# liannuaa/GenPC

Measured on AMD Instinct MI355X. Metric: chamfer_nn_pair_dist_throughput, higher is better.
Workload: dtype f32; 1 GPU; chamfer_3DDist.forward B=1 N=M=16384 (both directions), one pair per rank; points=16384, batch=1, arith=fma

## Files before the change

genpc_amd/csrc/nn.h:

```cpp
#pragma once
#include "common.h"
#include "grid.h"
#include "nn_plan.h"
#include "nn_decode.h"
#include "nn_ragged_dense_plan.h"

namespace genpc {

constexpr int kWavesPerBlock = kBlock / kWave;

struct NNDir {
    const unsigned *dupmask;
    float *tmaxp;
    unsigned long long *part;
    const float *q;
    const float *t;
    float *out_d;
    int *out_i;
    const uint4 *arec;
    int block_begin;
    int dup_shared;
    NNDiv by_qblocks;
    int qblocks;
    int nq, nt;
    int slices;
    int fin_begin;
    NNDiv by_fblocks;
    int ntmax;
    int unit_begin;
    int ntp;
};

struct NNArgs {
    NNDir dir[2];
    int slice_len;
    NNDiv by_b;
    int ndir;
    int b;
    int debug;
    int hint_stride;
    NNDiv by_hint;
    int fma;
    unsigned long long *stats;
    unsigned *hint;
    int *arrive;
    float radius2;
};

#define NN_GLOBAL(T) __attribute__((address_space(1))) T *
#define NN_CONST(p) ((const __attribute__((address_space(4))) float *)(p))
#define NN_ARG(T, name, field) T name##_0 = a.dir[0].field, name##_1 = a.dir[1].field
#define NN_ARG_PTR(T, name, field) NN_GLOBAL(T) name##_0 = (NN_GLOBAL(T))a.dir[0].field; NN_GLOBAL(T) name##_1 = (NN_GLOBAL(T))a.dir[1].field
#define NN_HELD(name) "+s"(name##_0), "+s"(name##_1)
#define NN_OF_DIR(name) (d ? name##_1 : name##_0)

typedef float f32x16 __attribute__((ext_vector_type(16)));

struct Top3 {
    float a1, a2, a3;
    int c1, c2;
};

__device__ __forceinline__ void top3_init(Top3 &s)
{
    s.a1 = s.a2 = s.a3 = __builtin_inff();
    s.c1 = s.c2 = -1;
}

__device__ __forceinline__ void top3_insert(Top3 &s, float m, int id)
{
    asm("v_cmp_lt_f32 vcc, %[m], %[a2]\n\t"
        "v_cndmask_b32 %[c2], %[c2], %[id], vcc\n\t"
        "v_cmp_lt_f32 vcc, %[m], %[a1]\n\t"
        "v_cndmask_b32 %[c2], %[c2], %[c1], vcc\n\t"
        "v_cndmask_b32 %[c1], %[c1], %[id], vcc\n\t"
        "v_med3_f32 %[a3], %[a2], %[a3], %[m]\n\t"
        "v_med3_f32 %[a2], %[a1], %[a2], %[m]\n\t"
        "v_min_f32 %[a1], %[a1], %[m]"
        : [a1] "+v"(s.a1), [a2] "+v"(s.a2), [a3] "+v"(s.a3), [c1] "+v"(s.c1), [c2] "+v"(s.c2)
        : [m] "v"(m), [id] "v"(id)
        : "vcc");
}

__device__ __forceinline__ unsigned list_enc(float base, float v)
{
    if (!(v < __builtin_inff())) return v != v ? 0xffffu : 0xff00u;
    const float s = fmaxf(fabsf(base), fabsf(v)) * 4.76837158203125e-07f;
    const float d = (v - base) - s;
    if (!(d > 0.0f)) return 0u;
    return (__float_as_uint(d) >> 15) & 0xffffu;
}
__device__ __forceinline__ float list_dec(float base, unsigned code) { return base + __uint_as_float(code << 15); }

typedef unsigned long long ListRec __attribute__((ext_vector_type(2)));
template <typename P>
__device__ __forceinline__ auto list_rec(P *part, int list, size_t bnq, int batch, int nq, int j)
{
    typedef typename std::conditional<std::is_const<P>::value, const ListRec, ListRec>::type R;
    return (R *)part + ((size_t)list * bnq + (size_t)batch * nq + j);
}

template <int FMA, int LEN>
__device__ __forceinline__ void rescan_chunk(const float *__restrict__ T, int nt, int base, float qx, float qy,
                                             float qz, float &bd, int &bi)
{
    typedef float f4u __attribute__((ext_vector_type(4), aligned(4)));
    bd = __builtin_inff();
    bi = base;
    if (base + LEN <= nt) {
        const f4u *tp = (const f4u *)(T + (size_t)base * 3);
#pragma unroll
        for (int c8 = LEN - 8; c8 >= 0; c8 -= 8) {
            f4u v[6];
#pragma unroll
            for (int i = 0; i < 6; i++) v[i] = tp[(c8 >> 2) * 3 + i];
            const float f[24] = {v[0].x, v[0].y, v[0].z, v[0].w, v[1].x, v[1].y, v[1].z, v[1].w,
                                 v[2].x, v[2].y, v[2].z, v[2].w, v[3].x, v[3].y, v[3].z, v[3].w,
                                 v[4].x, v[4].y, v[4].z, v[4].w, v[5].x, v[5].y, v[5].z, v[5].w};
#pragma unroll
            for (int c = 7; c >= 0; c--) {
                const float dd = sqdist<FMA>(f[c * 3 + 0] - qx, f[c * 3 + 1] - qy, f[c * 3 + 2] - qz);
                const bool le = dd <= bd;
                bd = le ? dd : bd;
                bi = le ? base + c8 + c : bi;
            }
        }
    } else {
        for (int c = LEN - 1; c >= 0; c--) {
            int kk = base + c;
            kk = kk < nt ? kk : nt - 1;
            const float *tp = T + (size_t)kk * 3;
            const float dd = sqdist<FMA>(tp[0] - qx, tp[1] - qy, tp[2] - qz);
            const bool le = dd <= bd;
            bd = le ? dd : bd;
            bi = le ? kk : bi;
        }
    }
}

__device__ __forceinline__ int tile_row(int w) { return 8 * ((w >> 2) & 3) + 4 * (w >> 4) + (w & 3); }

constexpr int kRefTile = 512;

__device__ __forceinline__ int block_or(int v, int *s)
{
    static_assert(kWavesPerBlock * kWave == kBlock, "block_or folds one word per wave of a kBlock-thread block");
    const int any = __ballot(v != 0) != 0ull;
    __syncthreads();
    if ((threadIdx.x & (kWave - 1)) == 0) s[threadIdx.x >> 6] = any;
    __syncthreads();
    int r = 0;
#pragma unroll
    for (int w = 0; w < kWavesPerBlock; w++) r |= s[w];
    return r;
}
template <int FMA>
__device__ __forceinline__ void nn_exhaustive(const float *__restrict__ Qp, const float *__restrict__ T, int nt, int j,
                                              float *__restrict__ od, int *__restrict__ oi, float *s_red, int *s_fi)
{
    const int lane = threadIdx.x & (kWave - 1), wave = threadIdx.x >> 6;
    const float x = Qp[(size_t)j * 3 + 0], y = Qp[(size_t)j * 3 + 1], z = Qp[(size_t)j * 3 + 2];
    int dead = 0;
    for (int k = threadIdx.x * kRefTile; k < nt; k += kBlock * kRefTile) {
        const float *tp = T + (size_t)k * 3;
        const float hd = sqdist<FMA>(tp[0] - x, tp[1] - y, tp[2] - z);
        dead |= hd != hd;
    }
    dead = block_or(dead, s_fi);
    float bd = __builtin_inff();
    int bi = 0x7fffffff;
    if (!dead) {
        for (int k = threadIdx.x; k < nt; k += kBlock) {
            const float *tp = T + (size_t)k * 3;
            const float dd = sqdist<FMA>(tp[0] - x, tp[1] - y, tp[2] - z);
            const bool lt = dd < bd;
            bd = lt ? dd : bd;
            bi = lt ? k : bi;
        }
    } else {
        for (int k = threadIdx.x; k < nt; k += kBlock) {
            const float *hp = T + (size_t)(k & ~(kRefTile - 1)) * 3;
            const float hd = sqdist<FMA>(hp[0] - x, hp[1] - y, hp[2] - z);
            const float *tp = T + (size_t)k * 3;
            const float dd = sqdist<FMA>(tp[0] - x, tp[1] - y, tp[2] - z);
            const bool lt = dd < bd && hd == hd;
            bd = lt ? dd : bd;
            bi = lt ? k : bi;
        }
    }
#pragma unroll
    for (int o = 32; o >= 1; o >>= 1) {
        const float obd = __shfl_xor(bd, o);
        const int obi = __shfl_xor(bi, o);
        const bool other = obd < bd || (obd == bd && obi < bi);
        bd = other ? obd : bd;
        bi = other ? obi : bi;
    }
    __syncthreads();
    if (lane == 0) { s_red[wave] = bd; s_fi[wave] = bi; }
    __syncthreads();
    if (threadIdx.x == 0) {
        for (int w = 1; w < kWavesPerBlock; w++) {
            const bool other = s_red[w] < bd || (s_red[w] == bd && s_fi[w] < bi);
            bd = other ? s_red[w] : bd;
            bi = other ? s_fi[w] : bi;
        }
        const float d0 = sqdist<FMA>(T[0] - x, T[1] - y, T[2] - z);
        if (d0 != d0 || bi == 0x7fffffff) {
            bd = d0;
            bi = 0;
        }
        od[j] = bd;
        oi[j] = bi;
    }
}

__device__ __forceinline__ float nn_tau(float a_best, float qq, float tmax2, double kQT, double kTT)
{
    const double u = 1.01 * 5.9604644775390625e-8;
    const double T = sqrt((double)tmax2), qn = sqrt((double)qq);
    const double kSub = 64.0 * 1.401298464324817e-45;
    const double E1 = u * (kQT * qn * T + kTT * T * T + 3.0 * (double)qq) + kSub;
    const double eta = u * (qn + T);
    double up = (double)a_best + (double)qq + E1;
    up = sqrt(up > 0.0 ? up : 0.0) + eta;
    up = up * up * (1.0 + 6.0 * u) + kSub;
    double r = sqrt(up / (1.0 - 6.0 * u)) + eta;
    const double tau = r * r - (double)qq + E1;
    float tf = (float)tau;
    if ((double)tf < tau) tf = __uint_as_float(__float_as_uint(tf) + (tf >= 0.0f ? 1 : -1));
    return tf;
}


constexpr int kHalfMin = 16;
typedef float f4u __attribute__((ext_vector_type(4), aligned(4)));
struct HalfPiece {
    f4u v[12];
};

__device__ __forceinline__ int half_window(int nt, int first) { return first < nt - 16 ? first : nt - 16; }

__device__ __forceinline__ void rescan_half_issue(const float *__restrict__ T, int nt, int base, int h, HalfPiece &p)
{
    const f4u *tp = (const f4u *)(T + (size_t)half_window(nt, base + 16 * h) * 3);
#pragma unroll
    for (int k = 0; k < 12; k++) p.v[k] = tp[k];
}

template <int FMA>
__device__ __forceinline__ void rescan_half_eval(const HalfPiece &p, int nt, int base, int h, float qx, float qy, float qz,
                                                 float &bd, int &bi)
{
    const int first = base + 16 * h, start = half_window(nt, first);
    const int skip = first - start < 15 ? first - start : 15;
    bd = __builtin_inff();
    int be = skip;
#pragma unroll
    for (int e = 15; e >= 0; e--) {
        const float dd = sqdist<FMA>(p.v[(e * 3) >> 2][(e * 3) & 3] - qx, p.v[(e * 3 + 1) >> 2][(e * 3 + 1) & 3] - qy,
                                     p.v[(e * 3 + 2) >> 2][(e * 3 + 2) & 3] - qz);
        const bool le = dd <= bd && e >= skip;
        bd = le ? dd : bd;
        be = le ? e : be;
    }
    bi = start + be;
}

template <int FMA>
__device__ __forceinline__ void rescan_half_small(const float *__restrict__ T, int nt, int base, int h, float qx, float qy,
                                                  float qz, float &bd, int &bi)
{
    const int first = base + 16 * h;
    bd = __builtin_inff();
    bi = first < nt ? first : nt - 1;
    for (int c = 15; c >= 0; c--) {
        int kk = first + c;
        kk = kk < nt ? kk : nt - 1;
        const float *tp = T + (size_t)kk * 3;
        const float dd = sqdist<FMA>(tp[0] - qx, tp[1] - qy, tp[2] - qz);
        const bool le = dd <= bd;
        bd = le ? dd : bd;
        bi = le ? kk : bi;
    }
}

template <int FMA>
__device__ __forceinline__ void rescan_half(const float *__restrict__ T, int nt, int base, int h, float qx, float qy,
                                            float qz, float &bd, int &bi)
{
    if (nt >= kHalfMin) {
        HalfPiece p;
        rescan_half_issue(T, nt, base, h, p);
        rescan_half_eval<FMA>(p, nt, base, h, qx, qy, qz, bd, bi);
    } else {
        rescan_half_small<FMA>(T, nt, base, h, qx, qy, qz, bd, bi);
    }
}

int launch_nn_f16(NNArgs &a, const NNPlan &plan, hipStream_t st);
int launch_nn_finish(const NNArgs &a, const NNPlan &plan, float kqt, float ktt, float t2min, hipStream_t st);
int launch_nn_grid(const NNArgs &a, hipStream_t st);
size_t nn_dedupe_mask_words(int b, int n);
int launch_nn_dedupe(int b, int nclouds, const float *const pts[2], const int n[2], unsigned *const masks[2], unsigned *hint,
                     hipStream_t st);
int nn_forward(int b, int ndir, const float *q0, int n0, const float *t0, int m0, float *d0, int *i0, const float *q1,
               int n1, const float *t1, int m1, float *d1, int *i1, hipStream_t st, float radius2 = __builtin_inff(),
               const unsigned *dup0 = nullptr, const unsigned *dup1 = nullptr, int dup_shared = 0);

struct SeededGrids {
    const CellGridHdr *hdr_static, *hdr_rest;
    const int *start_static, *start_rest;
    const float4 *sorted_static, *sorted_rest;
};
void seeded_grids_layout(WsLayout &L, SeededGrids &g, int b, int nm, int ns);
int build_seeded_grids(int b, int nm, const float *rest_pts, int ns, const float *static_pts, const SeededGrids &g, hipStream_t st);
int launch_nn_seeded(int b, int nm, const float *moving_pts, int ns, const float *static_pts, const SeededGrids &g, const float *center,
                     int cstride, const float *params, int pstride, float *d1, int *i1, float *d2, int *i2, int fma, hipStream_t st, int sample = 1);

struct NnRaggedGrids {
    const CellGridHdr *hdr;
    const int *start;
    const float4 *sorted;
};
void nn_ragged_grids_layout(WsLayout &L, NnRaggedGrids &g, const RaggedTable &t);
int nn_ragged_build(const RaggedTable &t, int max_targets, const float *xyz2, const NnRaggedGrids &g, hipStream_t st);
int nn_ragged_search(const RaggedTable &t, const float *xyz, const NnRaggedGrids &g, float *result, int *result_i, hipStream_t st);
int nn_ragged_dense(const RaggedTable &t, const float *queries, const float *targets, float *d, int *i, hipStream_t st);
extern thread_local int t_nn_ragged_dense;

}
```

genpc_amd/csrc/nn_f16.hip:

```cpp
#include "nn.h"
#include <hip/hip_ext.h>
#include "../../include/genpc_hip.h"

#include <stdlib.h>

namespace genpc {

typedef _Float16 h16x8 __attribute__((ext_vector_type(8)));

#ifdef GENPC_NN_TIMELINE
constexpr int kTimelineRow = 16;
__device__ unsigned long long g_timeline[4096 * kTimelineRow];
#define GENPC_TL(k) do { if (threadIdx.x == 0 && blockIdx.x < 4096) { g_timeline[blockIdx.x * kTimelineRow + (k)] = __builtin_readcyclecounter(); \
    if ((k) == 0) g_timeline[blockIdx.x * kTimelineRow + 6] = wall_clock64(); if ((k) == 5) g_timeline[blockIdx.x * kTimelineRow + 7] = wall_clock64(); } } while (0)
#define GENPC_TL_PARTNER(k) do { if (WV == 8 && threadIdx.x == 4 * kWave && blockIdx.x < 4096) g_timeline[blockIdx.x * kTimelineRow + (k)] = __builtin_readcyclecounter(); } while (0)
#else
#define GENPC_TL(k) do {} while (0)
#define GENPC_TL_PARTNER(k) do {} while (0)
#endif
constexpr double kQTh = 30.0, kTTh = 15.0;

__device__ __forceinline__ unsigned f16_bits(float v) { return (unsigned)__builtin_bit_cast(unsigned short, (_Float16)v); }

__device__ __forceinline__ unsigned split2(float v)
{
    const _Float16 h = (_Float16)v;
    const _Float16 l = (_Float16)(v - (float)h);
    return (unsigned)__builtin_bit_cast(unsigned short, h) | ((unsigned)__builtin_bit_cast(unsigned short, l) << 16);
}

__device__ __forceinline__ unsigned dup_lo(unsigned v) { return __builtin_amdgcn_perm(v, v, 0x01000100u); }
__device__ __forceinline__ unsigned dup_hi(unsigned v) { return __builtin_amdgcn_perm(v, v, 0x03020302u); }

__device__ __forceinline__ float scale_for(float m)
{
    if (!(m > 0.0f) || !(m < __builtin_inff())) return 1.0f;
    const int e = __builtin_amdgcn_frexp_expf(m);
    return __builtin_ldexpf(1.0f, 11 - e);
}

template <int Q, int U, int NL, int W, int HT, int WV>
__global__ __launch_bounds__(WV * kWave, W) void nn_f16_kernel(NNArgs a)
{
    constexpr int kThreads = WV * kWave;
    static_assert(Q >= 2, "one accumulator chain per wave violates the MFMA -> VALU wait states");
    constexpr int kC = 32 * U;
    constexpr int kRows = HT + 64;
    __shared__ uint4 plane[2][kRows];
    __shared__ float s_red[WV];
    GENPC_TL(0);
    const int lane = threadIdx.x & (kWave - 1);
    const int wave = threadIdx.x >> 6;
    const int half = lane >> 5, col = lane & 31;
    int ndir = a.ndir, nbatch = a.b, slice_len = a.slice_len, debug = a.debug;
    NNDiv by_b = a.by_b;
    NN_ARG(int, begin, block_begin); NN_ARG(int, qblocks, qblocks); NN_ARG(NNDiv, by_q, by_qblocks);
    NN_ARG(int, nq, nq); NN_ARG(int, nt, nt); NN_ARG(int, slices, slices); NN_ARG(int, dupsh, dup_shared);
    NN_ARG_PTR(const float, q, q); NN_ARG_PTR(const float, t, t); NN_ARG_PTR(const unsigned, dup, dupmask);
    NN_ARG_PTR(float, tmaxp, tmaxp); NN_ARG_PTR(unsigned long long, part, part);
    asm volatile("" : "+s"(ndir), "+s"(nbatch), "+s"(slice_len), "+s"(debug), "+s"(by_b.mul), "+s"(by_b.shift), NN_HELD(begin), NN_HELD(qblocks),
                 "+s"(by_q_0.mul), "+s"(by_q_0.shift), "+s"(by_q_1.mul), "+s"(by_q_1.shift), NN_HELD(nq), NN_HELD(nt), NN_HELD(slices), NN_HELD(dupsh),
                 NN_HELD(q), NN_HELD(t), NN_HELD(dup), NN_HELD(tmaxp), NN_HELD(part));
    const int d = (ndir > 1 && (int)blockIdx.x >= begin_1) ? 1 : 0;
    const int qblocks = NN_OF_DIR(qblocks), nq = NN_OF_DIR(nq), nt = NN_OF_DIR(nt), slices = NN_OF_DIR(slices), dup_shared = NN_OF_DIR(dupsh);
    const float *const q_dir = (const float *)NN_OF_DIR(q), *const t_dir = (const float *)NN_OF_DIR(t);
    const float *const t_dir0 = (const float *)t_0;
    const int nt_dir0 = nt_0;
    const unsigned *const dup_dir = (const unsigned *)NN_OF_DIR(dup);
    float *const tmaxp_dir = (float *)NN_OF_DIR(tmaxp);
    unsigned long long *const part_dir = (unsigned long long *)NN_OF_DIR(part);
    const NNBlockId id = nn_decode_block((int)blockIdx.x - NN_OF_DIR(begin), qblocks, NNDiv{NN_OF_DIR(by_q).mul, NN_OF_DIR(by_q).shift}, nbatch, by_b);
    const int qb = id.qb, batch = id.batch, slice = id.slice;

    const float *__restrict__ Qp = q_dir + (size_t)batch * nq * 3;
    const float *__restrict__ T = t_dir + (size_t)batch * nt * 3;
    const auto cptr = NN_CONST(t_dir0 + (size_t)batch * nt_dir0 * 3);
    const float cx = cptr[0], cy = cptr[1], cz = cptr[2];

    const int k_begin = slice * slice_len;
    int k_end = k_begin + slice_len;
    if (k_end > nt) k_end = nt;

    float raw0[Q], raw1[Q];
    const int q0 = (qb * WV + wave) * (32 * Q) + col;
    GENPC_TL(8);
#pragma unroll
    for (int r = 0; r < Q; r++) {
        int j = q0 + r * 32;
        if (j >= nq) j = nq - 1;
        raw0[r] = Qp[(size_t)j * 3 + (half ? 2 : 0)];
        raw1[r] = Qp[(size_t)j * 3 + 1];
    }
    constexpr int kPer = HT / kThreads;
    float pre[kPer][3];
    const unsigned *__restrict__ dupm = dup_dir ? dup_dir + (dup_shared ? (size_t)0 : (size_t)batch * ((nt + 31) >> 5)) : nullptr;
    unsigned predup = 0u;
    auto prefetch = [&](int t0) {
        predup = 0u;
        int tc[kPer];
#pragma unroll
        for (int i = 0; i < kPer; i++) {
            const int t = t0 + i * kThreads + threadIdx.x;
            tc[i] = t < nt ? t : nt - 1;
#pragma unroll
            for (int k = 0; k < 3; k++) pre[i][k] = T[(size_t)tc[i] * 3 + k];
        }
        if (dupm) {
            unsigned mw[kPer];
#pragma unroll
            for (int i = 0; i < kPer; i++) mw[i] = dupm[tc[i] >> 5];
#pragma unroll
            for (int i = 0; i < kPer; i++) predup |= ((mw[i] >> (tc[i] & 31)) & 1u) << i;
        }
    };
    const bool resident = k_end - k_begin <= HT;
    if (resident && k_begin < k_end) prefetch(k_begin);
    float qc0[Q], qc1[Q];
    float mx = 0.0f;
#pragma unroll
    for (int r = 0; r < Q; r++) {
        qc0[r] = raw0[r] - (half ? cz : cx);
        qc1[r] = half ? 0.0f : raw1[r] - cy;
        const float m0 = fabsf(qc0[r]), m1 = fabsf(qc1[r]);
        mx = fmaxf(mx, fmaxf(m0 < __builtin_inff() ? m0 : 0.0f, m1 < __builtin_inff() ? m1 : 0.0f));
    }
    if (resident) {
#pragma unroll
        for (int i = 0; i < kPer; i++)
            if (k_begin + i * kThreads + (int)threadIdx.x < k_end)
                mx = fmaxf(mx, fmaxf(fmaxf(fabsf(pre[i][0] - cx), fabsf(pre[i][1] - cy)), fabsf(pre[i][2] - cz)));
    } else {
        for (int t = k_begin + threadIdx.x; t < k_end; t += kThreads) {
            const float *tp = T + (size_t)t * 3;
            mx = fmaxf(mx, fmaxf(fmaxf(fabsf(tp[0] - cx), fabsf(tp[1] - cy)), fabsf(tp[2] - cz)));
        }
    }
#pragma unroll
    for (int o = 32; o >= 1; o >>= 1) mx = fmaxf(mx, __shfl_xor(mx, o));
    if (lane == 0) s_red[wave] = mx;
    __syncthreads();
    mx = s_red[0];
#pragma unroll
    for (int w2 = 1; w2 < WV; w2++) mx = fmaxf(mx, s_red[w2]);
    GENPC_TL(1);
    const float sc = scale_for(mx);
    const float isc = 1.0f / sc;
    const float tsc = -2.0f * sc;

    h16x8 bq[Q];
    Top3 lst[Q][NL];
#pragma unroll
    for (int r = 0; r < Q; r++) {
        const unsigned p0 = split2(qc0[r] * sc), p1 = split2(qc1[r] * sc);
        const uint4 v = half ? make_uint4(p0, p0, 0x5c005c00u, 0u) : make_uint4(p0, p0, p1, p1);
        bq[r] = __builtin_bit_cast(h16x8, v);
#pragma unroll
        for (int n = 0; n < NL; n++) top3_init(lst[r][n]);
    }

    f32x16 acc[Q];
    uint4 A[2];
    auto fetch = [&](int p, int row) { A[p] = plane[half][row + col]; };
    auto mm = [&](int p, int r) {
        const f32x16 z = {0.f, 0.f, 0.f, 0.f, 0.f, 0.f, 0.f, 0.f, 0.f, 0.f, 0.f, 0.f, 0.f, 0.f, 0.f, 0.f};
        acc[r] = __builtin_amdgcn_mfma_f32_32x32x16_f16(__builtin_bit_cast(h16x8, A[p]), bq[r], z, 0, 0, 0);
    };
    auto step = [&](auto p_tag, auto last_tag, int row, float (&m)[Q][4]) {
        constexpr int p = decltype(p_tag)::value;
        constexpr bool last = decltype(last_tag)::value;
        if (!last) fetch(p, row + 64);
        if (Q == 2) asm volatile("s_nop 3");
#pragma unroll
        for (int r = 0; r < Q; r++) {
            const f32x16 &c = acc[r];
            __builtin_amdgcn_sched_barrier(0);
#pragma unroll
            for (int e = 0; e < 16; e += 2)
                asm("v_min3_f32 %0, %1, %2, %3" : "=v"(m[r][(e >> 1) & 3]) : "v"(m[r][(e >> 1) & 3]), "v"(c[e]), "v"(c[e + 1]));
            __builtin_amdgcn_sched_barrier(0);
            if (!last) mm(p ^ 1, r);
            __builtin_amdgcn_sched_barrier(0);
        }
    };

    float tmax2 = 0.0f;
    float nf = 0.0f;
    if (!resident && k_begin < k_end) prefetch(k_begin);
    for (int t0 = k_begin; t0 < k_end && !(debug & 4); t0 += HT) {
        const int tn = min(HT, k_end - t0);
        const int tn_pad = (tn + kC - 1) / kC * kC;
        __syncthreads();
#pragma unroll
        for (int i = 0; i < kPer; i++) {
            const int t = i * kThreads + threadIdx.x;
            if (t < tn_pad) {
                const float x = pre[i][0] - cx, y = pre[i][1] - cy, z = pre[i][2] - cz;
                const float xs = x * sc, ys = y * sc, zs = z * sc;
                const float tts = __fmaf_rn(zs, zs, __fmaf_rn(ys, ys, __fmul_rn(xs, xs)));
                const unsigned px = split2(x * tsc), py = split2(y * tsc), pz = split2(z * tsc);
                const unsigned pt = split2(tts * 0.00390625f);
                uint4 V0 = make_uint4(dup_lo(px), dup_hi(px), dup_lo(py), dup_hi(py));
                uint4 V1 = make_uint4(dup_lo(pz), dup_hi(pz), pt, 0u);
                if (t >= tn || ((predup >> i) & 1u)) {
                    V0 = make_uint4(0u, 0u, 0u, 0u);
                    V1 = make_uint4(0u, 0u, 0x7c00u, 0u);
                } else {
                    const float tt = __fmaf_rn(z, z, __fmaf_rn(y, y, __fmul_rn(x, x)));
                    tmax2 = fmaxf(tmax2, tt);
                    nf = __fmaf_rn(tt, 0.0f, nf);
                }
                const int row = (t & ~31) | tile_row(t & 31);
                plane[0][row] = V0;
                plane[1][row] = V1;
            }
        }
        if (t0 + HT < k_end) prefetch(t0 + HT);
        __syncthreads();
        if (t0 == k_begin) { GENPC_TL(2); GENPC_TL_PARTNER(9); } else GENPC_TL(3);
        fetch(0, 0);
        fetch(1, 32);
#pragma unroll
        for (int r = 0; r < Q; r++) mm(0, r);
        asm volatile("s_nop 15");
        for (int rb0 = 0; rb0 < tn_pad; rb0 += NL * kC) {
#pragma unroll
            for (int n = 0; n < NL; n++) {
                const int rb = rb0 + n * kC;
                if (rb < tn_pad) {
                    float m[Q][4];
#pragma unroll
                    for (int r = 0; r < Q; r++) m[r][0] = m[r][1] = m[r][2] = m[r][3] = __builtin_inff();
#pragma unroll
                    for (int g = 0; g < U - 1; g++) {
                        if (g & 1) step(std::integral_constant<int, 1>{}, std::false_type{}, rb + 32 * g, m);
                        else step(std::integral_constant<int, 0>{}, std::false_type{}, rb + 32 * g, m);
                    }
                    if (rb + kC < tn_pad) step(std::integral_constant<int, 1>{}, std::false_type{}, rb + kC - 32, m);
                    else step(std::integral_constant<int, 1>{}, std::true_type{}, rb + kC - 32, m);
#pragma unroll
                    for (int r = 0; r < Q; r++) {
                        float v;
                        asm("v_min3_f32 %0, %1, %2, %3" : "=v"(v) : "v"(m[r][0]), "v"(m[r][1]), "v"(m[r][2]));
                        asm("v_min_f32 %0, %1, %2" : "=v"(v) : "v"(v), "v"(m[r][3]));
                        top3_insert(lst[r][n], v, t0 + rb + half);
                    }
                }
            }
        }
    }

    GENPC_TL(4);
    GENPC_TL_PARTNER(10);
    if (qb == 0) {
        if (nf != nf) tmax2 = __builtin_inff();
#pragma unroll
        for (int o = 32; o >= 1; o >>= 1) tmax2 = fmaxf(tmax2, __shfl_xor(tmax2, o));
        __syncthreads();
        if (lane == 0) s_red[wave] = tmax2;
        __syncthreads();
        float tm = s_red[0];
#pragma unroll
        for (int w2 = 1; w2 < WV; w2++) tm = fmaxf(tm, s_red[w2]);
        if (threadIdx.x == 0) tmaxp_dir[(size_t)batch * slices + slice] = tm;
    }

    const size_t bnq = (size_t)nbatch * nq;
#pragma unroll
    for (int r = 0; r < Q; r++) {
#pragma unroll
        for (int n = 0; n < NL; n++) {
            Top3 &f = lst[r][n];
            f.a1 = (f.a1 * isc) * isc;
            f.a2 = (f.a2 * isc) * isc;
            f.a3 = (f.a3 * isc) * isc;
            const float o1 = __shfl_xor(f.a1, 32), o2 = __shfl_xor(f.a2, 32), o3 = __shfl_xor(f.a3, 32);
            const int oc1 = __shfl_xor(f.c1, 32), oc2 = __shfl_xor(f.c2, 32);
            top3_insert(f, o1, oc1);
            top3_insert(f, o2, oc2);
            top3_insert(f, o3, -1);
            const int j = q0 + r * 32;
            if (!half && j < nq) {
                const unsigned code2 = list_enc(f.a1, f.a2);
                const unsigned code3 = list_enc(list_dec(f.a1, code2), f.a3);
                ListRec rec;
                rec.x = ((unsigned long long)__float_as_uint(f.a1) << 32) | (unsigned)f.c1;
                rec.y = ((unsigned long long)((code2 << 16) | code3) << 32) | (unsigned)f.c2;
                ListRec *p = list_rec(part_dir, slice * NL + n, bnq, batch, nq, j);
                asm volatile("global_store_dwordx4 %0, %1, off sc1\n\ts_nop 1" : : "v"((NN_GLOBAL(ListRec))p), "v"(rec) : "memory");
            }
        }
    }
    GENPC_TL(5);
    GENPC_TL_PARTNER(11);
}

template <int Q, int NL>
static void launch_main(const NNArgs &a, const NNPlan &plan, hipStream_t st, hipEvent_t e0, hipEvent_t e1)
{
#define NN_F16_LAUNCH(KERNEL, GRID, BLOCK)                                                                              \
    do {                                                                                                                \
        if (e0) hipExtLaunchKernelGGL(KERNEL, GRID, BLOCK, 0, st, e0, e1, 0, a);                                        \
        else hipLaunchKernelGGL(KERNEL, GRID, BLOCK, 0, st, a);                                                         \
    } while (0)
    const int blocks = (int)plan.blocks;
    if (Q == 4 && plan.form == kNNWide) {
        if (plan.unit == 2) NN_F16_LAUNCH((nn_f16_kernel<4, 2, NL, 1, 2 * kHTile, 8>), dim3(blocks), dim3(8 * kWave));
        else NN_F16_LAUNCH((nn_f16_kernel<4, 4, NL, 1, 2 * kHTile, 8>), dim3(blocks), dim3(8 * kWave));
    } else if (Q == 4 && plan.form == kNNTile2048) {
        if (plan.unit == 2) NN_F16_LAUNCH((nn_f16_kernel<4, 2, NL, 2, 2 * kHTile, 4>), dim3(blocks), dim3(kBlock));
        else NN_F16_LAUNCH((nn_f16_kernel<4, 4, NL, 2, 2 * kHTile, 4>), dim3(blocks), dim3(kBlock));
    } else if (Q == 4 && plan.form == kNNThreeWave) {
        if (plan.unit == 2) NN_F16_LAUNCH((nn_f16_kernel<Q, 2, NL, (Q == 4 ? 3 : 4), kHTile, 4>), dim3(blocks), dim3(kBlock));
        else NN_F16_LAUNCH((nn_f16_kernel<Q, 4, NL, (Q == 4 ? 3 : 4), kHTile, 4>), dim3(blocks), dim3(kBlock));
    } else {
        if (plan.unit == 2) NN_F16_LAUNCH((nn_f16_kernel<Q, 2, NL, (Q == 4 ? 2 : 4), kHTile, 4>), dim3(blocks), dim3(kBlock));
        else NN_F16_LAUNCH((nn_f16_kernel<Q, 4, NL, (Q == 4 ? 2 : 4), kHTile, 4>), dim3(blocks), dim3(kBlock));
    }
#undef NN_F16_LAUNCH
}

static thread_local bool g_prof_on = false;
static thread_local hipEvent_t g_prof_e0 = nullptr, g_prof_e1 = nullptr;

int launch_nn_f16(NNArgs &a, const NNPlan &plan, hipStream_t st)
{
    WsLayout L;
    for (int d = 0; d < a.ndir; d++) L.add(a.dir[d].tmaxp, (size_t)a.b * a.dir[d].ntmax);
    if (!ws_alloc(L, kWsNnTmax, st)) return 0;
    hipEvent_t pe0 = nullptr, pe1 = nullptr;
    if (g_prof_on) {
        if (!g_prof_e0) { (void)hipEventCreate(&g_prof_e0); (void)hipEventCreate(&g_prof_e1); }
        pe0 = g_prof_e0;
        pe1 = g_prof_e1;
    }
    if (plan.q == 4) {
        if (plan.nl == 2) launch_main<4, 2>(a, plan, st, pe0, pe1);
        else launch_main<4, 1>(a, plan, st, pe0, pe1);
    } else {
        if (plan.nl == 2) launch_main<2, 2>(a, plan, st, pe0, pe1);
        else launch_main<2, 1>(a, plan, st, pe0, pe1);
    }
    if (!check(hipGetLastError(), "nn_f16_kernel launch")) return 0;
    return launch_nn_finish(a, plan, (float)kQTh, (float)kTTh, 0.0f, st);
}

}

#ifdef GENPC_NN_TIMELINE
extern "C" __attribute__((visibility("default"))) int genpc_nn_timeline_read(unsigned long long *out)
{
    return hipMemcpyFromSymbol(out, HIP_SYMBOL(genpc::g_timeline), sizeof(unsigned long long) * 4096 * genpc::kTimelineRow) == hipSuccess;
}
#endif

GENPC_API float genpc_nn_profile(int enable)
{
    using namespace genpc;
    float ms = -1.0f;
    if (g_prof_on && g_prof_e1 && hipEventSynchronize(g_prof_e1) == hipSuccess) (void)hipEventElapsedTime(&ms, g_prof_e0, g_prof_e1);
    g_prof_on = enable != 0;
    return ms;
}
```

Measured before the change: 19010 Gpair-dist/s.

## Streamline point loads, full-tile staging, and halve epilogue merge work via permlane32 swap

Loads query and target points as packed 12-byte structs through 32-bit offsets from a uniform global base instead of per-component 64-bit indexed loads. Adds a fast path for full, duplicate-free tiles that skips per-row bounds and dup checks, and computes the tmax statistic only in blocks that publish it (qb==0). The epilogue now uses permlane32_swap so each lane half merges and stores a different half of the query tiles, instead of both halves merging and only one storing. Stores use scalar-base plus vector-offset addressing. This removes redundant ALU and address work in prologue and epilogue, at the cost of more code paths and a requirement that Q is even.

```diff
diff --git a/genpc_amd/csrc/nn.h b/genpc_amd/csrc/nn.h
--- a/genpc_amd/csrc/nn.h
+++ b/genpc_amd/csrc/nn.h
@@ -54,6 +54,14 @@
 #define NN_HELD(name) "+s"(name##_0), "+s"(name##_1)
 #define NN_OF_DIR(name) (d ? name##_1 : name##_0)
 
+struct NNPoint { float x, y, z; };
+__device__ __forceinline__ NNPoint nn_load_point(NN_GLOBAL(const char) base, unsigned bytes)
+{
+    NNPoint p;
+    __builtin_memcpy(&p, (const char *)(base + bytes), sizeof(NNPoint));
+    return p;
+}
+
 typedef float f32x16 __attribute__((ext_vector_type(16)));
 
 struct Top3 {
diff --git a/genpc_amd/csrc/nn_f16.hip b/genpc_amd/csrc/nn_f16.hip
--- a/genpc_amd/csrc/nn_f16.hip
+++ b/genpc_amd/csrc/nn_f16.hip
@@ -63,7 +63,7 @@
                  NN_HELD(q), NN_HELD(t), NN_HELD(dup), NN_HELD(tmaxp), NN_HELD(part));
     const int d = (ndir > 1 && (int)blockIdx.x >= begin_1) ? 1 : 0;
     const int qblocks = NN_OF_DIR(qblocks), nq = NN_OF_DIR(nq), nt = NN_OF_DIR(nt), slices = NN_OF_DIR(slices), dup_shared = NN_OF_DIR(dupsh);
-    const float *const q_dir = (const float *)NN_OF_DIR(q), *const t_dir = (const float *)NN_OF_DIR(t);
+    const float *const t_dir = (const float *)NN_OF_DIR(t);
     const float *const t_dir0 = (const float *)t_0;
     const int nt_dir0 = nt_0;
     const unsigned *const dup_dir = (const unsigned *)NN_OF_DIR(dup);
@@ -72,7 +72,6 @@
     const NNBlockId id = nn_decode_block((int)blockIdx.x - NN_OF_DIR(begin), qblocks, NNDiv{NN_OF_DIR(by_q).mul, NN_OF_DIR(by_q).shift}, nbatch, by_b);
     const int qb = id.qb, batch = id.batch, slice = id.slice;
 
-    const float *__restrict__ Qp = q_dir + (size_t)batch * nq * 3;
     const float *__restrict__ T = t_dir + (size_t)batch * nt * 3;
     const auto cptr = NN_CONST(t_dir0 + (size_t)batch * nt_dir0 * 3);
     const float cx = cptr[0], cy = cptr[1], cz = cptr[2];
@@ -82,19 +81,23 @@
     if (k_end > nt) k_end = nt;
 
     float raw0[Q], raw1[Q];
-    const int q0 = (qb * WV + wave) * (32 * Q) + col;
+    const int qfirst = qb * (WV * 32 * Q);
+    const int q0 = qfirst + wave * (32 * Q) + col;
+    const auto q_base = (NN_GLOBAL(const char))NN_OF_DIR(q) + ((size_t)batch * nq + qfirst) * sizeof(NNPoint);
     GENPC_TL(8);
 #pragma unroll
     for (int r = 0; r < Q; r++) {
         int j = q0 + r * 32;
         if (j >= nq) j = nq - 1;
-        raw0[r] = Qp[(size_t)j * 3 + (half ? 2 : 0)];
-        raw1[r] = Qp[(size_t)j * 3 + 1];
+        const NNPoint p = nn_load_point(q_base, (unsigned)(j - qfirst) * (unsigned)sizeof(NNPoint));
+        raw0[r] = half ? p.z : p.x;
+        raw1[r] = p.y;
     }
     constexpr int kPer = HT / kThreads;
     float pre[kPer][3];
     const unsigned *__restrict__ dupm = dup_dir ? dup_dir + (dup_shared ? (size_t)0 : (size_t)batch * ((nt + 31) >> 5)) : nullptr;
     unsigned predup = 0u;
+    const auto t_base = (NN_GLOBAL(const char))NN_OF_DIR(t) + (size_t)batch * nt * sizeof(NNPoint);
     auto prefetch = [&](int t0) {
         predup = 0u;
         int tc[kPer];
@@ -102,8 +105,10 @@
         for (int i = 0; i < kPer; i++) {
             const int t = t0 + i * kThreads + threadIdx.x;
             tc[i] = t < nt ? t : nt - 1;
-#pragma unroll
-            for (int k = 0; k < 3; k++) pre[i][k] = T[(size_t)tc[i] * 3 + k];
+            const NNPoint p = nn_load_point(t_base, (unsigned)tc[i] * (unsigned)sizeof(NNPoint));
+            pre[i][0] = p.x;
+            pre[i][1] = p.y;
+            pre[i][2] = p.z;
         }
         if (dupm) {
             unsigned mw[kPer];
@@ -114,6 +119,9 @@
         }
     };
     const bool resident = k_end - k_begin <= HT;
+    constexpr bool kStraight = !(W == 3 && NL == 2);
+    const bool full = kStraight && k_end - k_begin == HT && !dupm;
+    const bool publishes = qb == 0;
     if (resident && k_begin < k_end) prefetch(k_begin);
     float qc0[Q], qc1[Q];
     float mx = 0.0f;
@@ -124,7 +132,11 @@
         const float m0 = fabsf(qc0[r]), m1 = fabsf(qc1[r]);
         mx = fmaxf(mx, fmaxf(m0 < __builtin_inff() ? m0 : 0.0f, m1 < __builtin_inff() ? m1 : 0.0f));
     }
-    if (resident) {
+    if (full) {
+#pragma unroll
+        for (int i = 0; i < kPer; i++)
+            mx = fmaxf(mx, fmaxf(fmaxf(fabsf(pre[i][0] - cx), fabsf(pre[i][1] - cy)), fabsf(pre[i][2] - cz)));
+    } else if (resident) {
 #pragma unroll
         for (int i = 0; i < kPer; i++)
             if (k_begin + i * kThreads + (int)threadIdx.x < k_end)
@@ -190,31 +202,55 @@
         const int tn = min(HT, k_end - t0);
         const int tn_pad = (tn + kC - 1) / kC * kC;
         __syncthreads();
-#pragma unroll
-        for (int i = 0; i < kPer; i++) {
-            const int t = i * kThreads + threadIdx.x;
-            if (t < tn_pad) {
-                const float x = pre[i][0] - cx, y = pre[i][1] - cy, z = pre[i][2] - cz;
-                const float xs = x * sc, ys = y * sc, zs = z * sc;
-                const float tts = __fmaf_rn(zs, zs, __fmaf_rn(ys, ys, __fmul_rn(xs, xs)));
-                const unsigned px = split2(x * tsc), py = split2(y * tsc), pz = split2(z * tsc);
-                const unsigned pt = split2(tts * 0.00390625f);
-                uint4 V0 = make_uint4(dup_lo(px), dup_hi(px), dup_lo(py), dup_hi(py));
-                uint4 V1 = make_uint4(dup_lo(pz), dup_hi(pz), pt, 0u);
-                if (t >= tn || ((predup >> i) & 1u)) {
-                    V0 = make_uint4(0u, 0u, 0u, 0u);
-                    V1 = make_uint4(0u, 0u, 0x7c00u, 0u);
-                } else {
-                    const float tt = __fmaf_rn(z, z, __fmaf_rn(y, y, __fmul_rn(x, x)));
-                    tmax2 = fmaxf(tmax2, tt);
-                    nf = __fmaf_rn(tt, 0.0f, nf);
-                }
+        auto rows_of = [&](int i, uint4 &V0, uint4 &V1) {
+            const float x = pre[i][0] - cx, y = pre[i][1] - cy, z = pre[i][2] - cz;
+            const float xs = x * sc, ys = y * sc, zs = z * sc;
+            const float tts = __fmaf_rn(zs, zs, __fmaf_rn(ys, ys, __fmul_rn(xs, xs)));
+            const unsigned px = split2(x * tsc), py = split2(y * tsc), pz = split2(z * tsc);
+            const unsigned pt = split2(tts * 0.00390625f);
+            V0 = make_uint4(dup_lo(px), dup_hi(px), dup_lo(py), dup_hi(py));
+            V1 = make_uint4(dup_lo(pz), dup_hi(pz), pt, 0u);
+        };
+        auto measure = [&](int i) {
+            const float x = pre[i][0] - cx, y = pre[i][1] - cy, z = pre[i][2] - cz;
+            const float tt = __fmaf_rn(z, z, __fmaf_rn(y, y, __fmul_rn(x, x)));
+            tmax2 = fmaxf(tmax2, tt);
+            nf = __fmaf_rn(tt, 0.0f, nf);
+        };
+        if (full) {
+#pragma unroll
+            for (int i = 0; i < kPer; i++) {
+                const int t = i * kThreads + threadIdx.x;
+                uint4 V0, V1;
+                rows_of(i, V0, V1);
                 const int row = (t & ~31) | tile_row(t & 31);
                 plane[0][row] = V0;
                 plane[1][row] = V1;
             }
-        }
-        if (t0 + HT < k_end) prefetch(t0 + HT);
+            if (publishes) {
+#pragma unroll
+                for (int i = 0; i < kPer; i++) measure(i);
+            }
+        } else {
+#pragma unroll
+            for (int i = 0; i < kPer; i++) {
+                const int t = i * kThreads + threadIdx.x;
+                if (t < tn_pad) {
+                    uint4 V0, V1;
+                    rows_of(i, V0, V1);
+                    if (t >= tn || ((predup >> i) & 1u)) {
+                        V0 = make_uint4(0u, 0u, 0u, 0u);
+                        V1 = make_uint4(0u, 0u, 0x7c00u, 0u);
+                    } else if (publishes) {
+                        measure(i);
+                    }
+                    const int row = (t & ~31) | tile_row(t & 31);
+                    plane[0][row] = V0;
+                    plane[1][row] = V1;
+                }
+            }
+            if (t0 + HT < k_end) prefetch(t0 + HT);
+        }
         __syncthreads();
         if (t0 == k_begin) { GENPC_TL(2); GENPC_TL_PARTNER(9); } else GENPC_TL(3);
         fetch(0, 0);
@@ -251,7 +287,7 @@
 
     GENPC_TL(4);
     GENPC_TL_PARTNER(10);
-    if (qb == 0) {
+    if (publishes) {
         if (nf != nf) tmax2 = __builtin_inff();
 #pragma unroll
         for (int o = 32; o >= 1; o >>= 1) tmax2 = fmaxf(tmax2, __shfl_xor(tmax2, o));
@@ -265,28 +301,46 @@
     }
 
     const size_t bnq = (size_t)nbatch * nq;
-#pragma unroll
-    for (int r = 0; r < Q; r++) {
+    constexpr int QH = Q / 2;
+    static_assert(Q % 2 == 0, "the lane halves take half of the query tiles each");
+    auto swap_word = [](auto &a, auto &b) {
+        const auto v = __builtin_amdgcn_permlane32_swap(__builtin_bit_cast(unsigned, a), __builtin_bit_cast(unsigned, b), false, false);
+        const unsigned va = v[0], vb = v[1];
+        a = __builtin_bit_cast(std::remove_reference_t<decltype(a)>, va);
+        b = __builtin_bit_cast(std::remove_reference_t<decltype(b)>, vb);
+    };
+    auto swap_halves = [&](Top3 &a, Top3 &b) {
+        swap_word(a.a1, b.a1);
+        swap_word(a.a2, b.a2);
+        swap_word(a.a3, b.a3);
+        swap_word(a.c1, b.c1);
+        swap_word(a.c2, b.c2);
+    };
+#pragma unroll
+    for (int r = 0; r < QH; r++) {
 #pragma unroll
         for (int n = 0; n < NL; n++) {
-            Top3 &f = lst[r][n];
+            Top3 &f = lst[r][n], &o = lst[r + QH][n];
             f.a1 = (f.a1 * isc) * isc;
             f.a2 = (f.a2 * isc) * isc;
             f.a3 = (f.a3 * isc) * isc;
-            const float o1 = __shfl_xor(f.a1, 32), o2 = __shfl_xor(f.a2, 32), o3 = __shfl_xor(f.a3, 32);
-            const int oc1 = __shfl_xor(f.c1, 32), oc2 = __shfl_xor(f.c2, 32);
-            top3_insert(f, o1, oc1);
-            top3_insert(f, o2, oc2);
-            top3_insert(f, o3, -1);
-            const int j = q0 + r * 32;
-            if (!half && j < nq) {
+            o.a1 = (o.a1 * isc) * isc;
+            o.a2 = (o.a2 * isc) * isc;
+            o.a3 = (o.a3 * isc) * isc;
+            swap_halves(f, o);
+            top3_insert(f, o.a1, o.c1);
+            top3_insert(f, o.a2, o.c2);
+            top3_insert(f, o.a3, -1);
+            const int j = q0 + (r + QH * half) * 32;
+            if (j < nq) {
                 const unsigned code2 = list_enc(f.a1, f.a2);
                 const unsigned code3 = list_enc(list_dec(f.a1, code2), f.a3);
                 ListRec rec;
                 rec.x = ((unsigned long long)__float_as_uint(f.a1) << 32) | (unsigned)f.c1;
                 rec.y = ((unsigned long long)((code2 << 16) | code3) << 32) | (unsigned)f.c2;
-                ListRec *p = list_rec(part_dir, slice * NL + n, bnq, batch, nq, j);
-                asm volatile("global_store_dwordx4 %0, %1, off sc1\n\ts_nop 1" : : "v"((NN_GLOBAL(ListRec))p), "v"(rec) : "memory");
+                ListRec *p = list_rec(part_dir, slice * NL + n, bnq, batch, nq, qfirst);
+                asm volatile("global_store_dwordx4 %0, %1, %2 sc1\n\ts_nop 1"
+                             : : "v"((unsigned)(j - qfirst) * (unsigned)sizeof(ListRec)), "v"(rec), "s"((NN_GLOBAL(ListRec))p) : "memory");
             }
         }
     }
```

After: 19920 Gpair-dist/s, median of 6. 1.05x the previous value.
